# yewzijian/RegTR

Measured on AMD Instinct MI355X. Metric: point-cloud pairs/sec (3DMatch ~20k pts), higher is better.
Workload: dtype f32 (f16-pair split, 22-bit operands)

## Files before the change

### regtr_amd/csrc/block_tail.hip

```cpp
#include "common.h"
#include "mfma_operands.h"

namespace {


constexpr int MO_WAVES = 4;
constexpr int MO_ROWS_WAVE = 512;
constexpr int MO_ROWS_WG = MO_WAVES * MO_ROWS_WAVE;

template <int KC, bool INFOLD, bool ROWDIV>
__global__ void __launch_bounds__(MO_WAVES* RG_WAVE, 4) k_moments(const float* __restrict__ A, int lda, const float2* __restrict__ stats,
                                                               float slope, const float* __restrict__ row_div, int k_valid,
                                                               const int* __restrict__ seg_off, int n_chunks,
                                                               double* __restrict__ partial, float* __restrict__ pivot)
{
    constexpr int K = 32 * KC, NTILE = KC * (KC + 1) / 2;
    __shared__ double red[K * K + K];
    const int cloud = blockIdx.y, chunk = blockIdx.x;
    const int c_end = seg_off[cloud + 1];
    const int wg_begin = seg_off[cloud] + chunk * MO_ROWS_WG;
    if (wg_begin >= c_end) return;
    const int lane = rg_lane(), wave = __builtin_amdgcn_readfirstlane(threadIdx.x >> 6);
    const int half = lane >> 5, ch = lane & 31;
    const bool ch_ok = ch < k_valid;
    const int chc = ch_ok ? ch : 0;
    const int w_begin = wg_begin + wave * MO_ROWS_WAVE, w_end = min(c_end, w_begin + MO_ROWS_WAVE);
    float mu[KC], rs[KC];
#pragma unroll
    for (int c = 0; c < KC; c++) {
        mu[c] = 0.f; rs[c] = 1.f;
        if (INFOLD) { const float2 s = stats[(size_t)cloud * K + 32 * c + chc]; mu[c] = s.x; rs[c] = s.y; }
    }
    float pv[KC];
    {
        const int r0 = seg_off[cloud];
        const long long n_c = c_end - r0;
        float v16[16][KC], d16[ROWDIV ? 16 : 1];
#pragma unroll
        for (int i = 0; i < 16; i++) {
            const int row = r0 + (int)(((2 * i + 1) * n_c) >> 5);
#pragma unroll
            for (int c = 0; c < KC; c++) v16[i][c] = A[(size_t)row * lda + 32 * c + chc];
            if (ROWDIV) d16[i] = row_div[row];
        }
#pragma unroll
        for (int c = 0; c < KC; c++) {
            float acc16 = 0.f, lo = 3.0e38f, hi = -3.0e38f;
#pragma unroll
            for (int i = 0; i < 16; i++) {
                float v = v16[i][c];
                if (ROWDIV) v = v / d16[ROWDIV ? i : 0];
                if (INFOLD) { const float u = (v - mu[c]) * rs[c]; v = fmaxf(u, u * slope); }
                acc16 += v; lo = fminf(lo, v); hi = fmaxf(hi, v);
            }
            pv[c] = ch_ok ? (acc16 - lo - hi) * (1.f / 14.f) : 0.f;
        }
    }
    floatx16 acc[NTILE];
    float s1[KC];
#pragma unroll
    for (int t = 0; t < NTILE; t++)
#pragma unroll
        for (int r = 0; r < 16; r++) acc[t][r] = 0.f;
#pragma unroll
    for (int c = 0; c < KC; c++) s1[c] = 0.f;
    constexpr int SUB = 16;
    constexpr int DS = ROWDIV ? SUB : 1;
    auto load = [&](float (&xv)[SUB][KC], float (&dv)[DS], int base) {
#pragma unroll
        for (int s = 0; s < SUB; s++) {
            const int row = base + 2 * s + half;
            const int rcl = row < w_end ? row : w_end - 1;
            const float* ap = A + (size_t)rcl * lda + chc;
#pragma unroll
            for (int c = 0; c < KC; c++) xv[s][c] = ap[32 * c];
            if (ROWDIV) dv[s] = row_div[rcl];
        }
    };
    auto consume = [&](const float (&xv)[SUB][KC], const float (&dv)[DS], int base) {
#pragma unroll
        for (int s = 0; s < SUB; s++) {
            const bool ok = base + 2 * s + half < w_end && ch_ok;
            float x[KC];
#pragma unroll
            for (int c = 0; c < KC; c++) {
                float v = xv[s][c];
                if (ROWDIV) v = v / dv[ROWDIV ? s : 0];
                if (INFOLD) { const float u = (v - mu[c]) * rs[c]; v = fmaxf(u, u * slope); }
                x[c] = ok ? v - pv[c] : 0.f;
                s1[c] += x[c];
            }
            int t = 0;
#pragma unroll
            for (int ta = 0; ta < KC; ta++)
#pragma unroll
                for (int tb = ta; tb < KC; tb++, t++)
                    acc[t] = __builtin_amdgcn_mfma_f32_32x32x2f32(x[ta], x[tb], acc[t], 0, 0, 0);
        }
    };
    float xa[SUB][KC], xb[SUB][KC], da[DS], db[DS];
    if (w_begin < w_end) load(xa, da, w_begin);
    for (int base = w_begin; base < w_end; base += 4 * SUB) {
        load(xb, db, base + 2 * SUB);
        consume(xa, da, base);
        load(xa, da, base + 4 * SUB);
        consume(xb, db, base + 2 * SUB);
    }
    for (int w = 0; w < MO_WAVES; w++) {
        if (wave == w && w_begin < w_end) {
            int t = 0;
#pragma unroll
            for (int ta = 0; ta < KC; ta++)
#pragma unroll
                for (int tb = ta; tb < KC; tb++, t++)
#pragma unroll
                    for (int r = 0; r < 16; r++) {
                        const int a = 32 * ta + (r & 3) + 8 * (r >> 2) + 4 * half, b = 32 * tb + ch;
                        const double v = (w == 0 ? 0.0 : red[a * K + b]) + (double)acc[t][r];
                        red[a * K + b] = v;
                    }
#pragma unroll
            for (int c = 0; c < KC; c++) {
                const double v = (double)s1[c] + (double)__shfl_xor(s1[c], 32, RG_WAVE);
                if (half == 0) red[K * K + 32 * c + ch] = (w == 0 ? 0.0 : red[K * K + 32 * c + ch]) + v;
            }
        }
        __syncthreads();
    }
    const int kv = k_valid;
    double* out = partial + ((size_t)cloud * n_chunks + chunk) * (kv * kv + kv);
    for (int i = threadIdx.x; i < kv * kv + kv; i += MO_WAVES * RG_WAVE) {
        int src = K * K + (i - kv * kv);
        if (i < kv * kv) { const int a = i / kv, b = i - a * kv; src = a * K + b; }
        out[i] = red[src];
    }
    if (chunk == 0 && wave == 0 && half == 0 && ch_ok) {
#pragma unroll
        for (int c = 0; c < KC; c++) pivot[(size_t)cloud * kv + 32 * c + ch] = pv[c];
    }
}

template <int K>
__device__ void bt_prepare_source(const double* __restrict__ partial, int n_chunks_total, int n_valid, int n_rows, int cloud,
                                  const float* __restrict__ W_kn, int N, int col0, float eps, double* cov ,
                                  double2* quad , uint16_t* __restrict__ planes, float* __restrict__ in_mean,
                                  float2* __restrict__ out_stats, const float* __restrict__ pivot)
{
    const double inv_n = 1.0 / (double)n_rows;
    for (int i = threadIdx.x; i < K * K + K; i += blockDim.x) {
        int src = i;
        if (i < K * K) {
            const int a = i / K, b = i - a * K;
            if ((a >> 5) > (b >> 5)) src = b * K + a;
        }
        double s = 0.0;
        for (int c = 0; c < n_valid; c++) s += partial[((size_t)cloud * n_chunks_total + c) * (K * K + K) + src];
        cov[i] = s * inv_n;
    }
    __syncthreads();
    for (int i = threadIdx.x; i < K * K; i += blockDim.x) {
        const int a = i / K, b = i - a * K;
        cov[i] -= cov[K * K + a] * cov[K * K + b];
    }
    __syncthreads();
    if (threadIdx.x < K) {
        cov[K * K + threadIdx.x] += (double)pivot[(size_t)cloud * K + threadIdx.x];
        if (col0 == 0) in_mean[(size_t)cloud * K + threadIdx.x] = (float)cov[K * K + threadIdx.x];
    }
    __syncthreads();
    const int j = col0 + (threadIdx.x & 63), h = threadIdx.x >> 6;
    float wj[K];
#pragma unroll
    for (int a = 0; a < K; a++) wj[a] = W_kn[(size_t)a * N + j];
    double mean = 0.0, var = 0.0;
#pragma unroll 1
    for (int a = h * (K / 4); a < (h + 1) * (K / 4); a++) {
        double t = 0.0;
#pragma unroll
        for (int b = 0; b < K; b++) t += cov[a * K + b] * (double)wj[b];
        const double wa = (double)W_kn[(size_t)a * N + j];
        mean += cov[K * K + a] * wa;
        var += wa * t;
    }
    quad[threadIdx.x] = make_double2(mean, var);
    __syncthreads();
    {
        const int c = threadIdx.x & 63;
        const double2 q0 = quad[c], q1 = quad[64 + c], q2 = quad[128 + c], q3 = quad[192 + c];
        mean = (q0.x + q1.x) + (q2.x + q3.x);
        var = (q0.y + q1.y) + (q2.y + q3.y);
    }
    if (var < 0.0) var = 0.0;
    const float rstd = (float)(1.0 / sqrt(var + (double)eps));
    if (out_stats && h == 0) out_stats[(size_t)cloud * N + j] = make_float2((float)mean, rstd);
    uint16_t* row = planes + ((size_t)cloud * 3 * N + j) * K;
    for (int k = h * (K / 4); k < (h + 1) * (K / 4); k += 2) {
        unsigned p0, p1, p2;
        rg_split2(W_kn[(size_t)k * N + j] * rstd, W_kn[(size_t)(k + 1) * N + j] * rstd, p0, p1, p2);
        *(unsigned*)(row + k) = p0;
        *(unsigned*)(row + (size_t)N * K + k) = p1;
        *(unsigned*)(row + (size_t)2 * N * K + k) = p2;
    }
    __syncthreads();
}

template <int K1, int K2>
__global__ void __launch_bounds__(256) k_tail_prepare(const double* __restrict__ part1, const double* __restrict__ part2,
                                                      const int* __restrict__ seg_off, int n_chunks, const float* __restrict__ W1,
                                                      const float* __restrict__ W2, int N, float eps, uint16_t* __restrict__ planes1,
                                                      uint16_t* __restrict__ planes2, float* __restrict__ mean1,
                                                      float* __restrict__ mean2, float2* __restrict__ out_stats, int n_clouds,
                                                      const float* __restrict__ pivot1, const float* __restrict__ pivot2)
{
    constexpr int KM = K1 > K2 ? K1 : K2;
    __shared__ double cov[KM * KM + KM];
    __shared__ double2 quad[256];
    const int cloud = blockIdx.x, col0 = blockIdx.y * 64;
    const int n = seg_off[cloud + 1] - seg_off[cloud];
    if (n <= 0) {
        if (out_stats && threadIdx.x < 64) {
            out_stats[(size_t)cloud * N + col0 + threadIdx.x] = make_float2(0.f, 0.f);
            if (K2 > 0) out_stats[((size_t)n_clouds + cloud) * N + col0 + threadIdx.x] = make_float2(0.f, 0.f);
        }
        return;
    }
    const int n_valid = (n + MO_ROWS_WG - 1) / MO_ROWS_WG;
    bt_prepare_source<K1>(part1, n_chunks, n_valid, n, cloud, W1, N, col0, eps, cov, quad, planes1, mean1, out_stats, pivot1);
    if constexpr (K2 > 0)
        bt_prepare_source<K2>(part2, n_chunks, n_valid, n, cloud, W2, N, col0, eps, cov, quad, planes2, mean2,
                              out_stats ? out_stats + (size_t)n_clouds * N : nullptr, pivot2);
}

constexpr int TS_WAVES = 8;
constexpr int TS_ROWS = 32 * TS_WAVES;

struct TailArgs {
    const float* A1; const float* A2; float* Y;
    const float2* a1_stats;
    const float* row_div1;
    const float* mean1; const float* mean2;
    const uint16_t* planes1; const uint16_t* planes2;
    const int* seg_off; const int4* tile_info;
    int M, N, lda1, lda2, ldy, n_seg;
    float a1_slope, slope;
};

template <int KT> __device__ __forceinline__ unsigned ts_swz(unsigned n)
{
    constexpr int CPR = 2 * KT;
    return CPR == 2 ? 0u : (CPR == 4 ? ((n >> 2) & 3u) : (CPR == 8 ? ((n >> 1) & 7u) : (n & 15u)));
}

template <int KT, int NB>
__device__ __forceinline__ void ts_copy_planes(const uint16_t* __restrict__ src , size_t plane,
                                               unsigned char* dst, int t)
{
    constexpr int CPR = 2 * KT, K = 16 * KT, NDMA = 3 * NB * CPR / RG_WAVE;
    static_assert(3 * NB * CPR % RG_WAVE == 0, "whole DMA instructions");
    const int wave = __builtin_amdgcn_readfirstlane(t >> 6), lane = t & 63;
#pragma unroll 1
    for (int q0 = 0; q0 < NDMA; q0 += TS_WAVES) {
        const int q = q0 + wave;
        if (q < NDMA) {
            const int sidx = q * RG_WAVE + lane;
            const int p = sidx / (NB * CPR), rem = sidx - p * (NB * CPR), n = rem / CPR, cs = rem - n * CPR;
            __builtin_amdgcn_global_load_lds((const void*)(src + (size_t)p * plane + (size_t)n * K + (((unsigned)cs ^ ts_swz<KT>((unsigned)n)) * 8)),
                                             (rg_lds_ptr)(dst + (size_t)q * 1024), 16, 0, 0);
        }
    }
}

template <int KT1, int KT2, int NT, int NPASS, bool FOLD1>
__global__ void __launch_bounds__(TS_WAVES* RG_WAVE, NT <= 2 ? 4 : 2) k_tail_strip(TailArgs g)
{
    constexpr int K1 = 16 * KT1, K2 = 16 * KT2, NB = 32 * NT * NPASS, KT2A = KT2 > 0 ? KT2 : 1;
    extern __shared__ __align__(16) unsigned char Ws[];
    unsigned char* Ws2 = Ws + (size_t)3 * NB * K1 * 2;
    const int t = threadIdx.x, lane = t & 63, l31 = lane & 31, hi = lane >> 5;
    const int wave = __builtin_amdgcn_readfirstlane(t >> 6);
    const int N = g.N, n0 = blockIdx.y * NB;
    const int m0 = blockIdx.x * TS_ROWS, r0 = m0 + 32 * wave;
    const int row = r0 + l31;
    const bool row_ok = row < g.M;
    const int rc = row_ok ? row : g.M - 1;

    float4 raw1[KT1][2], raw2[KT2A][2];
    float div1 = 1.f;
    {
        const float* ap = g.A1 + (size_t)rc * g.lda1 + 8 * hi;
#pragma unroll
        for (int ks = 0; ks < KT1; ks++) { raw1[ks][0] = *(const float4*)(ap + 16 * ks); raw1[ks][1] = *(const float4*)(ap + 16 * ks + 4); }
        if constexpr (KT2 > 0) {
            const float* bp = g.A2 + (size_t)rc * g.lda2 + 8 * hi;
#pragma unroll
            for (int ks = 0; ks < KT2; ks++) { raw2[ks][0] = *(const float4*)(bp + 16 * ks); raw2[ks][1] = *(const float4*)(bp + 16 * ks + 4); }
        }
        if (!FOLD1 && g.row_div1) div1 = g.row_div1[rc];
    }
    const int4 ti = g.tile_info[blockIdx.x];
    const int s_lo = ti.x, s_hi = ti.y;
    ts_copy_planes<KT1, NB>(g.planes1 + ((size_t)s_lo * 3 * N + n0) * K1, (size_t)N * K1, Ws, t);
    if constexpr (KT2 > 0) ts_copy_planes<KT2, NB>(g.planes2 + ((size_t)s_lo * 3 * N + n0) * K2, (size_t)N * K2, Ws2, t);
    const int my_seg = s_lo == s_hi ? s_lo : rg_find_segment(g.seg_off, g.n_seg, rc);
    __syncthreads();

    {
        const float* mp = g.mean1 + (size_t)my_seg * K1 + 8 * hi;
        if constexpr (FOLD1) {
            const float2* sp = g.a1_stats + (size_t)my_seg * K1 + 8 * hi;
#pragma unroll
            for (int ks = 0; ks < KT1; ks++)
#pragma unroll
                for (int h = 0; h < 2; h++) {
                    const float4 sa = *(const float4*)(sp + 16 * ks + 4 * h), sb = *(const float4*)(sp + 16 * ks + 4 * h + 2);
                    const float4 m = *(const float4*)(mp + 16 * ks + 4 * h);
                    float4 v = raw1[ks][h];
                    float u;
                    u = (v.x - sa.x) * sa.y; v.x = row_ok ? fmaxf(u, u * g.a1_slope) - m.x : 0.f;
                    u = (v.y - sa.z) * sa.w; v.y = row_ok ? fmaxf(u, u * g.a1_slope) - m.y : 0.f;
                    u = (v.z - sb.x) * sb.y; v.z = row_ok ? fmaxf(u, u * g.a1_slope) - m.z : 0.f;
                    u = (v.w - sb.z) * sb.w; v.w = row_ok ? fmaxf(u, u * g.a1_slope) - m.w : 0.f;
                    raw1[ks][h] = v;
                }
        } else {
#pragma unroll
            for (int ks = 0; ks < KT1; ks++)
#pragma unroll
                for (int h = 0; h < 2; h++) {
                    const float4 m = *(const float4*)(mp + 16 * ks + 4 * h);
                    float4 v = raw1[ks][h];
                    if (g.row_div1) { v.x = v.x / div1; v.y = v.y / div1; v.z = v.z / div1; v.w = v.w / div1; }
                    v.x = row_ok ? v.x - m.x : 0.f; v.y = row_ok ? v.y - m.y : 0.f; v.z = row_ok ? v.z - m.z : 0.f; v.w = row_ok ? v.w - m.w : 0.f;
                    raw1[ks][h] = v;
                }
        }
        if constexpr (KT2 > 0) {
            const float* mq = g.mean2 + (size_t)my_seg * K2 + 8 * hi;
#pragma unroll
            for (int ks = 0; ks < KT2; ks++)
#pragma unroll
                for (int h = 0; h < 2; h++) {
                    const float4 m = *(const float4*)(mq + 16 * ks + 4 * h);
                    float4 v = raw2[ks][h];
                    v.x = row_ok ? v.x - m.x : 0.f; v.y = row_ok ? v.y - m.y : 0.f; v.z = row_ok ? v.z - m.z : 0.f; v.w = row_ok ? v.w - m.w : 0.f;
                    raw2[ks][h] = v;
                }
        }
    }
    auto frag = [&](const float4 (&r)[2], bf16x8 (&fa)[3]) {
        unsigned w[4][3];
        rg_split2(r[0].x, r[0].y, w[0]);
        rg_split2(r[0].z, r[0].w, w[1]);
        rg_split2(r[1].x, r[1].y, w[2]);
        rg_split2(r[1].z, r[1].w, w[3]);
#pragma unroll
        for (int p = 0; p < 3; p++) fa[p] = __builtin_bit_cast(bf16x8, make_uint4(w[0][p], w[1][p], w[2][p], w[3][p]));
    };
    unsigned f1_off[KT1], f2_off[KT2A];
#pragma unroll
    for (int ks = 0; ks < KT1; ks++) f1_off[ks] = (unsigned)l31 * (K1 * 2) + (((unsigned)(2 * ks + hi)) ^ ts_swz<KT1>((unsigned)l31)) * 16u;
    if constexpr (KT2 > 0) {
#pragma unroll
        for (int ks = 0; ks < KT2; ks++) f2_off[ks] = (unsigned)l31 * (K2 * 2) + (((unsigned)(2 * ks + hi)) ^ ts_swz<KT2A>((unsigned)l31)) * 16u;
    }

    const int rbase = r0 + 4 * hi;
    for (int sg = s_lo; sg <= s_hi; sg++) {
        if (sg > s_lo) {
            __syncthreads();
            ts_copy_planes<KT1, NB>(g.planes1 + ((size_t)sg * 3 * N + n0) * K1, (size_t)N * K1, Ws, t);
            if constexpr (KT2 > 0) ts_copy_planes<KT2, NB>(g.planes2 + ((size_t)sg * 3 * N + n0) * K2, (size_t)N * K2, Ws2, t);
            __syncthreads();
        }
        const int c_lo = sg == s_lo ? ti.z : g.seg_off[sg], c_hi = min(sg == s_lo ? ti.w : g.seg_off[sg + 1], g.M);
#pragma unroll 1
        for (int ps = 0; ps < NPASS; ps++) {
            const int cb = 32 * NT * ps;
            floatx16 acc[NT];
#pragma unroll
            for (int j = 0; j < NT; j++)
#pragma unroll
                for (int r = 0; r < 16; r++) acc[j][r] = 0.f;
#define TS_STEP(FA, WS_, OFF, KK)                                                                                            \
            _Pragma("unroll") for (int j = 0; j < NT; j++) {                                                                   \
                bf16x8 fb[3];                                                                                                  \
                _Pragma("unroll") for (int p = 0; p < 3; p++)                                                                  \
                    fb[p] = __builtin_bit_cast(bf16x8, *(const uint4*)(WS_ + (size_t)(p * NB + cb + 32 * j) * (KK * 2) + OFF)); \
                acc[j] = __builtin_amdgcn_mfma_f32_32x32x16_bf16(FA[2], fb[0], acc[j], 0, 0, 0);                               \
                acc[j] = __builtin_amdgcn_mfma_f32_32x32x16_bf16(FA[1], fb[1], acc[j], 0, 0, 0);                               \
                acc[j] = __builtin_amdgcn_mfma_f32_32x32x16_bf16(FA[0], fb[2], acc[j], 0, 0, 0);                               \
                acc[j] = __builtin_amdgcn_mfma_f32_32x32x16_bf16(FA[1], fb[0], acc[j], 0, 0, 0);                               \
                acc[j] = __builtin_amdgcn_mfma_f32_32x32x16_bf16(FA[0], fb[1], acc[j], 0, 0, 0);                               \
                acc[j] = __builtin_amdgcn_mfma_f32_32x32x16_bf16(FA[0], fb[0], acc[j], 0, 0, 0);                               \
            }
#pragma unroll
            for (int ks = 0; ks < KT1; ks++) { bf16x8 fa[3]; frag(raw1[ks], fa); TS_STEP(fa, Ws, f1_off[ks], K1) }
            if constexpr (KT2 > 0) {
#pragma unroll
                for (int ks = 0; ks < KT2; ks++) { bf16x8 fa[3]; frag(raw2[ks], fa); TS_STEP(fa, Ws2, f2_off[ks], K2) }
            }
#undef TS_STEP
            int rb = rbase;
            asm volatile("" : "+v"(rb));
#pragma unroll
            for (int j = 0; j < NT; j++) {
                const int col = n0 + cb + 32 * j + l31;
#pragma unroll
                for (int r = 0; r < 16; r++) {
                    const int rw = rb + (r & 3) + 8 * (r >> 2);
                    const float v = acc[j][r];
                    if (rw >= c_lo && rw < c_hi) g.Y[(size_t)rw * g.ldy + col] = fmaxf(v, v * g.slope);
                }
            }
        }
    }
}

int bt_chunks(int max_len) { return rg_cdiv(max_len > 0 ? max_len : 1, MO_ROWS_WG); }
size_t bt_align(size_t b) { return (b + 255) & ~(size_t)255; }

}

extern "C" {

int regtr_block_tail_supported(int M, int N, int K1, int K2)
{
    return (M >= 0 && ((K1 == 32 && K2 == 64 && N == 128) || (K1 == 16 && K2 == 0 && N == 64))) ? 1 : 0;
}

size_t regtr_block_tail_ws_bytes(int n_clouds, int max_len, int N, int K1, int K2)
{
    if (n_clouds < 1 || !regtr_block_tail_supported(0, N, K1, K2)) return 0;
    const size_t nc = (size_t)bt_chunks(max_len);
    return bt_align(n_clouds * nc * (K1 * K1 + K1) * 8) + bt_align(n_clouds * nc * (K2 * K2 + K2) * 8) +
           bt_align((size_t)n_clouds * 3 * N * K1 * 2) + bt_align((size_t)n_clouds * 3 * N * K2 * 2) +
           2 * (bt_align((size_t)n_clouds * K1 * 4) + bt_align((size_t)n_clouds * K2 * 4));
}

int regtr_block_tail(const float* A1, int lda1, const float* a1_stats, float a1_slope, const float* row_div1, const float* A2, int lda2,
                     const float* W1, const float* W2, const int* seg_off, int n_clouds, int max_len, const void* tile_info,
                     int M, int N, int K1, int K2, float eps, float slope, float* Y, int ldy, void* ws, size_t ws_bytes,
                     float* out_stats, void* stream)
{
    if (!A1 || !W1 || !seg_off || !tile_info || !Y || !ws || n_clouds < 1 || max_len < 0) return RG_ERR_ARG;
    if (!regtr_block_tail_supported(M, N, K1, K2) || lda1 < K1 || ldy < N || (lda1 % 4)) return RG_ERR_ARG;
    if (K2 > 0 && (!A2 || !W2 || !a1_stats || row_div1 || lda2 < K2 || (lda2 % 4) || (uintptr_t)A2 % 16)) return RG_ERR_ARG;
    if (K2 == 0 && (A2 || W2 || a1_stats || !row_div1)) return RG_ERR_ARG;
    if (((uintptr_t)A1 | (uintptr_t)a1_stats | (uintptr_t)tile_info | (uintptr_t)ws) % 16) return RG_ERR_ARG;
    if (ws_bytes < regtr_block_tail_ws_bytes(n_clouds, max_len, N, K1, K2)) return RG_ERR_WORKSPACE;
    if (M == 0 || max_len == 0) return RG_OK;
    const int nc = bt_chunks(max_len);
    unsigned char* p = (unsigned char*)ws;
    double* part1 = (double*)p; p += bt_align((size_t)n_clouds * nc * (K1 * K1 + K1) * 8);
    double* part2 = (double*)p; p += bt_align((size_t)n_clouds * nc * (K2 * K2 + K2) * 8);
    uint16_t* planes1 = (uint16_t*)p; p += bt_align((size_t)n_clouds * 3 * N * K1 * 2);
    uint16_t* planes2 = (uint16_t*)p; p += bt_align((size_t)n_clouds * 3 * N * K2 * 2);
    float* mean1 = (float*)p; p += bt_align((size_t)n_clouds * K1 * 4);
    float* mean2 = (float*)p; p += bt_align((size_t)n_clouds * K2 * 4);
    float* pivot1 = (float*)p; p += bt_align((size_t)n_clouds * K1 * 4);
    float* pivot2 = (float*)p;
    hipStream_t st = (hipStream_t)stream;
    const dim3 mgrid(nc, n_clouds), pgrid(n_clouds, N / 64), sgrid(rg_cdiv(M, TS_ROWS), 1);
    TailArgs g{A1, A2, Y, (const float2*)a1_stats, row_div1, mean1, mean2, planes1, planes2, seg_off, (const int4*)tile_info,
               M, N, lda1, lda2, ldy, n_clouds, a1_slope, slope};
    const size_t lds = (size_t)3 * N * (K1 + K2) * 2;
    if (K2 > 0) {
        k_moments<1, true, false><<<mgrid, MO_WAVES * RG_WAVE, 0, st>>>(A1, lda1, (const float2*)a1_stats, a1_slope, nullptr, K1, seg_off, nc, part1, pivot1);
        k_moments<2, false, false><<<mgrid, MO_WAVES * RG_WAVE, 0, st>>>(A2, lda2, nullptr, 0.f, nullptr, K2, seg_off, nc, part2, pivot2);
        k_tail_prepare<32, 64><<<pgrid, 256, 0, st>>>(part1, part2, seg_off, nc, W1, W2, N, eps, planes1, planes2, mean1, mean2,
                                                      (float2*)out_stats, n_clouds, pivot1, pivot2);
        if (!rg_allow_dynamic_lds<k_tail_strip<2, 4, 2, 2, true>>(lds)) return RG_ERR_ARG;
        k_tail_strip<2, 4, 2, 2, true><<<sgrid, TS_WAVES * RG_WAVE, lds, st>>>(g);
    } else {
        k_moments<1, false, true><<<mgrid, MO_WAVES * RG_WAVE, 0, st>>>(A1, lda1, nullptr, 0.f, row_div1, K1, seg_off, nc, part1, pivot1);
        k_tail_prepare<16, 0><<<pgrid, 256, 0, st>>>(part1, nullptr, seg_off, nc, W1, nullptr, N, eps, planes1, nullptr, mean1, nullptr,
                                                     (float2*)out_stats, n_clouds, pivot1, nullptr);
        if (!rg_allow_dynamic_lds<k_tail_strip<1, 0, 2, 1, false>>(lds)) return RG_ERR_ARG;
        k_tail_strip<1, 0, 2, 1, false><<<sgrid, TS_WAVES * RG_WAVE, lds, st>>>(g);
    }
    RG_RETURN_IF_LAUNCH_FAILED();
    return RG_OK;
}


}
```

Measured before the change: 2290.

## Stage moment inputs through LDS with float4 loads and parallel cross-wave reduction

The moments kernel now loads rows as coalesced float4 vectors into a per-wave LDS stage, applying the normalisation transform once per element, and then reads MFMA operands from LDS. The serial wave-by-wave double reduction is replaced by parking accumulators in LDS and having each wave reduce one slice across waves in parallel. The prepare kernel switches to one 512-thread block per cloud with register-blocked covariance quadratic forms. This trades extra LDS traffic and more LDS use for fewer strided global loads and less serialized reduction, and it hardcodes the column count (k_valid removed).

```diff
diff --git a/regtr_amd/csrc/block_tail.hip b/regtr_amd/csrc/block_tail.hip
--- a/regtr_amd/csrc/block_tail.hip
+++ b/regtr_amd/csrc/block_tail.hip
@@ -8,53 +8,96 @@
 constexpr int MO_ROWS_WAVE = 512;
 constexpr int MO_ROWS_WG = MO_WAVES * MO_ROWS_WAVE;
 
+__device__ __forceinline__ void mo_wave_sync()
+{
+    __builtin_amdgcn_fence(__ATOMIC_RELEASE, "wavefront");
+    __builtin_amdgcn_wave_barrier();
+    __builtin_amdgcn_fence(__ATOMIC_ACQUIRE, "wavefront");
+}
+
 template <int KC, bool INFOLD, bool ROWDIV>
-__global__ void __launch_bounds__(MO_WAVES* RG_WAVE, 4) k_moments(const float* __restrict__ A, int lda, const float2* __restrict__ stats,
-                                                               float slope, const float* __restrict__ row_div, int k_valid,
+__global__ void __launch_bounds__(MO_WAVES* RG_WAVE, KC == 1 ? 4 : 3) k_moments(const float* __restrict__ A, int lda, const float2* __restrict__ stats,
+                                                               float slope, const float* __restrict__ row_div,
                                                                const int* __restrict__ seg_off, int n_chunks,
                                                                double* __restrict__ partial, float* __restrict__ pivot)
 {
+    static_assert(!ROWDIV || KC == 1, "the row_div form has 16 columns");
     constexpr int K = 32 * KC, NTILE = KC * (KC + 1) / 2;
-    __shared__ double red[K * K + K];
+    constexpr int KV = ROWDIV ? 16 : K;
+    constexpr int CPR = KV / 4, RPI = RG_WAVE / CPR;
+    constexpr int NLD = 8, SUBR = NLD * RPI;
+    constexpr int GRP = 8 / KC;
+    constexpr int STAGE_F = SUBR * KV, PARK_F = NTILE * 16 * RG_WAVE, WAVE_F = STAGE_F > PARK_F ? STAGE_F : PARK_F;
+    __shared__ __align__(16) float lds[MO_WAVES * WAVE_F];
+    __shared__ double s1_park[MO_WAVES * K];
     const int cloud = blockIdx.y, chunk = blockIdx.x;
-    const int c_end = seg_off[cloud + 1];
-    const int wg_begin = seg_off[cloud] + chunk * MO_ROWS_WG;
+    const int r0 = seg_off[cloud], c_end = seg_off[cloud + 1];
+    const int wg_begin = r0 + chunk * MO_ROWS_WG;
     if (wg_begin >= c_end) return;
     const int lane = rg_lane(), wave = __builtin_amdgcn_readfirstlane(threadIdx.x >> 6);
     const int half = lane >> 5, ch = lane & 31;
-    const bool ch_ok = ch < k_valid;
-    const int chc = ch_ok ? ch : 0;
+    const bool ch_ok = ch < KV;
+    const int chr = ch & (KV - 1);
+    const int lrow = lane / CPR, lcol = 4 * (lane % CPR);
     const int w_begin = wg_begin + wave * MO_ROWS_WAVE, w_end = min(c_end, w_begin + MO_ROWS_WAVE);
-    float mu[KC], rs[KC];
-#pragma unroll
-    for (int c = 0; c < KC; c++) {
-        mu[c] = 0.f; rs[c] = 1.f;
-        if (INFOLD) { const float2 s = stats[(size_t)cloud * K + 32 * c + chc]; mu[c] = s.x; rs[c] = s.y; }
-    }
+    float* stage = lds + wave * WAVE_F;
+    float mu[4], rs[4];
+#pragma unroll
+    for (int q = 0; q < 4; q++) { mu[q] = 0.f; rs[q] = 1.f; }
+    if (INFOLD) {
+        const float4* sp = (const float4*)(stats + (size_t)cloud * K + lcol);
+        const float4 sa = sp[0], sb = sp[1];
+        mu[0] = sa.x; rs[0] = sa.y; mu[1] = sa.z; rs[1] = sa.w; mu[2] = sb.x; rs[2] = sb.y; mu[3] = sb.z; rs[3] = sb.w;
+    }
+    auto xform = [&](float4 v, float d) {
+        float x[4] = {v.x, v.y, v.z, v.w};
+#pragma unroll
+        for (int q = 0; q < 4; q++) {
+            if (ROWDIV) x[q] = x[q] / d;
+            if (INFOLD) { const float u = (x[q] - mu[q]) * rs[q]; x[q] = fmaxf(u, u * slope); }
+        }
+        return make_float4(x[0], x[1], x[2], x[3]);
+    };
+    float4 buf[NLD];
+    float dv[ROWDIV ? NLD : 1];
+    auto load = [&](int base) {
+#pragma unroll
+        for (int j = 0; j < NLD; j++) {
+            const int row = base + j * RPI + lrow;
+            const int rcl = row < w_end ? row : w_end - 1;
+            buf[j] = *(const float4*)(A + (size_t)rcl * lda + lcol);
+            if (ROWDIV) dv[j] = row_div[rcl];
+        }
+    };
+    if (w_begin < w_end) load(w_begin);
     float pv[KC];
-    {
-        const int r0 = seg_off[cloud];
+#pragma unroll
+    for (int c = 0; c < KC; c++) pv[c] = 0.f;
+    if (w_begin < w_end) {
         const long long n_c = c_end - r0;
-        float v16[16][KC], d16[ROWDIV ? 16 : 1];
-#pragma unroll
-        for (int i = 0; i < 16; i++) {
-            const int row = r0 + (int)(((2 * i + 1) * n_c) >> 5);
-#pragma unroll
-            for (int c = 0; c < KC; c++) v16[i][c] = A[(size_t)row * lda + 32 * c + chc];
-            if (ROWDIV) d16[i] = row_div[row];
-        }
+        constexpr int NS = 16 * CPR / RG_WAVE;
+        float4 sv[NS];
+        float sd[NS];
+#pragma unroll
+        for (int j = 0; j < NS; j++) {
+            const int row = r0 + (int)(((2 * (j * RPI + lrow) + 1) * n_c) >> 5);
+            sv[j] = *(const float4*)(A + (size_t)row * lda + lcol);
+            sd[j] = ROWDIV ? row_div[row] : 1.f;
+        }
+#pragma unroll
+        for (int j = 0; j < NS; j++) *(float4*)(stage + (j * RPI + lrow) * KV + lcol) = xform(sv[j], sd[j]);
+        mo_wave_sync();
 #pragma unroll
         for (int c = 0; c < KC; c++) {
             float acc16 = 0.f, lo = 3.0e38f, hi = -3.0e38f;
 #pragma unroll
             for (int i = 0; i < 16; i++) {
-                float v = v16[i][c];
-                if (ROWDIV) v = v / d16[ROWDIV ? i : 0];
-                if (INFOLD) { const float u = (v - mu[c]) * rs[c]; v = fmaxf(u, u * slope); }
+                const float v = stage[i * KV + 32 * c + chr];
                 acc16 += v; lo = fminf(lo, v); hi = fmaxf(hi, v);
             }
             pv[c] = ch_ok ? (acc16 - lo - hi) * (1.f / 14.f) : 0.f;
         }
+        mo_wave_sync();
     }
     floatx16 acc[NTILE];
     float s1[KC];
@@ -64,170 +107,198 @@
         for (int r = 0; r < 16; r++) acc[t][r] = 0.f;
 #pragma unroll
     for (int c = 0; c < KC; c++) s1[c] = 0.f;
-    constexpr int SUB = 16;
-    constexpr int DS = ROWDIV ? SUB : 1;
-    auto load = [&](float (&xv)[SUB][KC], float (&dv)[DS], int base) {
-#pragma unroll
-        for (int s = 0; s < SUB; s++) {
-            const int row = base + 2 * s + half;
-            const int rcl = row < w_end ? row : w_end - 1;
-            const float* ap = A + (size_t)rcl * lda + chc;
-#pragma unroll
-            for (int c = 0; c < KC; c++) xv[s][c] = ap[32 * c];
-            if (ROWDIV) dv[s] = row_div[rcl];
-        }
-    };
-    auto consume = [&](const float (&xv)[SUB][KC], const float (&dv)[DS], int base) {
-#pragma unroll
-        for (int s = 0; s < SUB; s++) {
-            const bool ok = base + 2 * s + half < w_end && ch_ok;
-            float x[KC];
-#pragma unroll
-            for (int c = 0; c < KC; c++) {
-                float v = xv[s][c];
-                if (ROWDIV) v = v / dv[ROWDIV ? s : 0];
-                if (INFOLD) { const float u = (v - mu[c]) * rs[c]; v = fmaxf(u, u * slope); }
-                x[c] = ok ? v - pv[c] : 0.f;
-                s1[c] += x[c];
-            }
-            int t = 0;
-#pragma unroll
-            for (int ta = 0; ta < KC; ta++)
-#pragma unroll
-                for (int tb = ta; tb < KC; tb++, t++)
-                    acc[t] = __builtin_amdgcn_mfma_f32_32x32x2f32(x[ta], x[tb], acc[t], 0, 0, 0);
-        }
-    };
-    float xa[SUB][KC], xb[SUB][KC], da[DS], db[DS];
-    if (w_begin < w_end) load(xa, da, w_begin);
-    for (int base = w_begin; base < w_end; base += 4 * SUB) {
-        load(xb, db, base + 2 * SUB);
-        consume(xa, da, base);
-        load(xa, da, base + 4 * SUB);
-        consume(xb, db, base + 2 * SUB);
-    }
-    for (int w = 0; w < MO_WAVES; w++) {
-        if (wave == w && w_begin < w_end) {
-            int t = 0;
-#pragma unroll
-            for (int ta = 0; ta < KC; ta++)
-#pragma unroll
-                for (int tb = ta; tb < KC; tb++, t++)
-#pragma unroll
-                    for (int r = 0; r < 16; r++) {
-                        const int a = 32 * ta + (r & 3) + 8 * (r >> 2) + 4 * half, b = 32 * tb + ch;
-                        const double v = (w == 0 ? 0.0 : red[a * K + b]) + (double)acc[t][r];
-                        red[a * K + b] = v;
+    for (int base = w_begin; base < w_end; base += SUBR) {
+#pragma unroll
+        for (int j = 0; j < NLD; j++) *(float4*)(stage + (j * RPI + lrow) * KV + lcol) = xform(buf[j], ROWDIV ? dv[ROWDIV ? j : 0] : 1.f);
+        mo_wave_sync();
+        if (base + SUBR < w_end) load(base + SUBR);
+        for (int s0 = 0; s0 < SUBR / 2 && base + 2 * s0 < w_end; s0 += GRP) {
+            float xv[GRP][KC];
+#pragma unroll
+            for (int s = 0; s < GRP; s++)
+#pragma unroll
+                for (int c = 0; c < KC; c++) xv[s][c] = stage[(2 * (s0 + s) + half) * KV + 32 * c + chr];
+#pragma unroll
+            for (int s = 0; s < GRP; s++)
+#pragma unroll
+                for (int c = 0; c < KC; c++) asm volatile("" : "+v"(xv[s][c]));
+#pragma unroll
+            for (int s = s0; s < s0 + GRP; s++) {
+                const bool ok = base + 2 * s + half < w_end && ch_ok;
+                float x[KC];
+#pragma unroll
+                for (int c = 0; c < KC; c++) {
+                    x[c] = ok ? xv[s - s0][c] - pv[c] : 0.f;
+                    s1[c] += x[c];
+                }
+                int t = 0;
+#pragma unroll
+                for (int ta = 0; ta < KC; ta++)
+#pragma unroll
+                    for (int tb = ta; tb < KC; tb++, t++)
+                        acc[t] = __builtin_amdgcn_mfma_f32_32x32x2f32(x[ta], x[tb], acc[t], 0, 0, 0);
+            }
+        }
+        mo_wave_sync();
+    }
+    if (w_begin < w_end) {
+#pragma unroll
+        for (int t = 0; t < NTILE; t++)
+#pragma unroll
+            for (int g = 0; g < 4; g++)
+                ((float4*)stage)[(t * 4 + g) * RG_WAVE + lane] = make_float4(acc[t][4 * g], acc[t][4 * g + 1], acc[t][4 * g + 2], acc[t][4 * g + 3]);
+#pragma unroll
+        for (int c = 0; c < KC; c++) {
+            const double v = (double)s1[c] + (double)__shfl_xor(s1[c], 32, RG_WAVE);
+            if (half == 0) s1_park[wave * K + 32 * c + ch] = v;
+        }
+    }
+    __syncthreads();
+    const int n_act = min(MO_WAVES, (c_end - wg_begin + MO_ROWS_WAVE - 1) / MO_ROWS_WAVE);
+    double* out = partial + ((size_t)cloud * n_chunks + chunk) * (KV * KV + KV);
+    {
+        const int g = wave;
+        int t = 0;
+#pragma unroll
+        for (int ta = 0; ta < KC; ta++)
+#pragma unroll
+            for (int tb = ta; tb < KC; tb++, t++) {
+                double sum[4] = {0.0, 0.0, 0.0, 0.0};
+#pragma unroll
+                for (int w = 0; w < MO_WAVES; w++)
+                    if (w < n_act) {
+                        const float4 v = ((const float4*)(lds + w * WAVE_F))[(t * 4 + g) * RG_WAVE + lane];
+                        sum[0] += (double)v.x; sum[1] += (double)v.y; sum[2] += (double)v.z; sum[3] += (double)v.w;
                     }
-#pragma unroll
-            for (int c = 0; c < KC; c++) {
-                const double v = (double)s1[c] + (double)__shfl_xor(s1[c], 32, RG_WAVE);
-                if (half == 0) red[K * K + 32 * c + ch] = (w == 0 ? 0.0 : red[K * K + 32 * c + ch]) + v;
-            }
-        }
-        __syncthreads();
-    }
-    const int kv = k_valid;
-    double* out = partial + ((size_t)cloud * n_chunks + chunk) * (kv * kv + kv);
-    for (int i = threadIdx.x; i < kv * kv + kv; i += MO_WAVES * RG_WAVE) {
-        int src = K * K + (i - kv * kv);
-        if (i < kv * kv) { const int a = i / kv, b = i - a * kv; src = a * K + b; }
-        out[i] = red[src];
+                const int a = 32 * ta + 8 * g + 4 * half, b = 32 * tb + ch;
+#pragma unroll
+                for (int q = 0; q < 4; q++)
+                    if (a + q < KV && b < KV) out[(size_t)(a + q) * KV + b] = sum[q];
+            }
+    }
+    if (threadIdx.x < KV) {
+        double s = 0.0;
+        for (int w = 0; w < n_act; w++) s += s1_park[w * K + threadIdx.x];
+        out[KV * KV + threadIdx.x] = s;
     }
     if (chunk == 0 && wave == 0 && half == 0 && ch_ok) {
 #pragma unroll
-        for (int c = 0; c < KC; c++) pivot[(size_t)cloud * kv + 32 * c + ch] = pv[c];
-    }
-}
+        for (int c = 0; c < KC; c++) pivot[(size_t)cloud * KV + 32 * c + ch] = pv[c];
+    }
+}
+
+constexpr int PR_THREADS = 512;
+constexpr int PR_MAX_N = 128;
 
 template <int K>
 __device__ void bt_prepare_source(const double* __restrict__ partial, int n_chunks_total, int n_valid, int n_rows, int cloud,
-                                  const float* __restrict__ W_kn, int N, int col0, float eps, double* cov ,
+                                  const float* __restrict__ W_kn, int N, float eps, double* cov ,
                                   double2* quad , uint16_t* __restrict__ planes, float* __restrict__ in_mean,
                                   float2* __restrict__ out_stats, const float* __restrict__ pivot)
 {
+    constexpr int NEL = K * K + K, NE = (NEL + PR_THREADS - 1) / PR_THREADS;
     const double inv_n = 1.0 / (double)n_rows;
-    for (int i = threadIdx.x; i < K * K + K; i += blockDim.x) {
-        int src = i;
-        if (i < K * K) {
-            const int a = i / K, b = i - a * K;
-            if ((a >> 5) > (b >> 5)) src = b * K + a;
-        }
-        double s = 0.0;
-        for (int c = 0; c < n_valid; c++) s += partial[((size_t)cloud * n_chunks_total + c) * (K * K + K) + src];
-        cov[i] = s * inv_n;
-    }
-    __syncthreads();
-    for (int i = threadIdx.x; i < K * K; i += blockDim.x) {
+    {
+        const double* pc = partial + (size_t)cloud * n_chunks_total * NEL;
+        int src[NE];
+        double s[NE];
+#pragma unroll
+        for (int e = 0; e < NE; e++) {
+            const int i = threadIdx.x + e * PR_THREADS;
+            src[e] = i < NEL ? i : 0;
+            if (i < K * K) {
+                const int a = i / K, b = i - a * K;
+                if ((a >> 5) > (b >> 5)) src[e] = b * K + a;
+            }
+            s[e] = 0.0;
+        }
+        for (int c = 0; c < n_valid; c++)
+#pragma unroll
+            for (int e = 0; e < NE; e++) s[e] += pc[(size_t)c * NEL + src[e]];
+#pragma unroll
+        for (int e = 0; e < NE; e++) {
+            const int i = threadIdx.x + e * PR_THREADS;
+            if (i < NEL) cov[i] = s[e] * inv_n;
+        }
+    }
+    __syncthreads();
+    for (int i = threadIdx.x; i < K * K; i += PR_THREADS) {
         const int a = i / K, b = i - a * K;
         cov[i] -= cov[K * K + a] * cov[K * K + b];
     }
     __syncthreads();
     if (threadIdx.x < K) {
         cov[K * K + threadIdx.x] += (double)pivot[(size_t)cloud * K + threadIdx.x];
-        if (col0 == 0) in_mean[(size_t)cloud * K + threadIdx.x] = (float)cov[K * K + threadIdx.x];
-    }
-    __syncthreads();
-    const int j = col0 + (threadIdx.x & 63), h = threadIdx.x >> 6;
-    float wj[K];
-#pragma unroll
-    for (int a = 0; a < K; a++) wj[a] = W_kn[(size_t)a * N + j];
-    double mean = 0.0, var = 0.0;
+        in_mean[(size_t)cloud * K + threadIdx.x] = (float)cov[K * K + threadIdx.x];
+    }
+    __syncthreads();
+    for (int item = threadIdx.x; item < 4 * N; item += PR_THREADS) {
+        const int h = item / N, j = item - h * N;
+        float wj[K];
+#pragma unroll
+        for (int a = 0; a < K; a++) wj[a] = W_kn[(size_t)a * N + j];
+        double mean = 0.0, var = 0.0;
 #pragma unroll 1
-    for (int a = h * (K / 4); a < (h + 1) * (K / 4); a++) {
-        double t = 0.0;
-#pragma unroll
-        for (int b = 0; b < K; b++) t += cov[a * K + b] * (double)wj[b];
-        const double wa = (double)W_kn[(size_t)a * N + j];
-        mean += cov[K * K + a] * wa;
-        var += wa * t;
-    }
-    quad[threadIdx.x] = make_double2(mean, var);
-    __syncthreads();
-    {
-        const int c = threadIdx.x & 63;
-        const double2 q0 = quad[c], q1 = quad[64 + c], q2 = quad[128 + c], q3 = quad[192 + c];
-        mean = (q0.x + q1.x) + (q2.x + q3.x);
-        var = (q0.y + q1.y) + (q2.y + q3.y);
-    }
-    if (var < 0.0) var = 0.0;
-    const float rstd = (float)(1.0 / sqrt(var + (double)eps));
-    if (out_stats && h == 0) out_stats[(size_t)cloud * N + j] = make_float2((float)mean, rstd);
-    uint16_t* row = planes + ((size_t)cloud * 3 * N + j) * K;
-    for (int k = h * (K / 4); k < (h + 1) * (K / 4); k += 2) {
-        unsigned p0, p1, p2;
-        rg_split2(W_kn[(size_t)k * N + j] * rstd, W_kn[(size_t)(k + 1) * N + j] * rstd, p0, p1, p2);
-        *(unsigned*)(row + k) = p0;
-        *(unsigned*)(row + (size_t)N * K + k) = p1;
-        *(unsigned*)(row + (size_t)2 * N * K + k) = p2;
+        for (int a0 = h * (K / 4); a0 < (h + 1) * (K / 4); a0 += 4) {
+            double t[4] = {0.0, 0.0, 0.0, 0.0};
+#pragma unroll
+            for (int b = 0; b < K; b++)
+#pragma unroll
+                for (int u = 0; u < 4; u++) t[u] = fma(cov[(a0 + u) * K + b], (double)wj[b], t[u]);
+#pragma unroll
+            for (int u = 0; u < 4; u++) {
+                const double wa = (double)W_kn[(size_t)(a0 + u) * N + j];
+                mean = fma(cov[K * K + a0 + u], wa, mean);
+                var = fma(wa, t[u], var);
+            }
+        }
+        quad[item] = make_double2(mean, var);
+    }
+    __syncthreads();
+    for (int item = threadIdx.x; item < 4 * N; item += PR_THREADS) {
+        const int h = item / N, j = item - h * N;
+        const double2 q0 = quad[j], q1 = quad[N + j], q2 = quad[2 * N + j], q3 = quad[3 * N + j];
+        const double mean = (q0.x + q1.x) + (q2.x + q3.x);
+        double var = (q0.y + q1.y) + (q2.y + q3.y);
+        if (var < 0.0) var = 0.0;
+        const float rstd = (float)(1.0 / sqrt(var + (double)eps));
+        if (out_stats && h == 0) out_stats[(size_t)cloud * N + j] = make_float2((float)mean, rstd);
+        uint16_t* row = planes + ((size_t)cloud * 3 * N + j) * K;
+        for (int k = h * (K / 4); k < (h + 1) * (K / 4); k += 2) {
+            unsigned p0, p1, p2;
+            rg_split2(W_kn[(size_t)k * N + j] * rstd, W_kn[(size_t)(k + 1) * N + j] * rstd, p0, p1, p2);
+            *(unsigned*)(row + k) = p0;
+            *(unsigned*)(row + (size_t)N * K + k) = p1;
+            *(unsigned*)(row + (size_t)2 * N * K + k) = p2;
+        }
     }
     __syncthreads();
 }
 
 template <int K1, int K2>
-__global__ void __launch_bounds__(256) k_tail_prepare(const double* __restrict__ part1, const double* __restrict__ part2,
-                                                      const int* __restrict__ seg_off, int n_chunks, const float* __restrict__ W1,
-                                                      const float* __restrict__ W2, int N, float eps, uint16_t* __restrict__ planes1,
-                                                      uint16_t* __restrict__ planes2, float* __restrict__ mean1,
-                                                      float* __restrict__ mean2, float2* __restrict__ out_stats, int n_clouds,
-                                                      const float* __restrict__ pivot1, const float* __restrict__ pivot2)
+__global__ void __launch_bounds__(PR_THREADS) k_tail_prepare(const double* __restrict__ part1, const double* __restrict__ part2,
+                                                             const int* __restrict__ seg_off, int n_chunks, const float* __restrict__ W1,
+                                                             const float* __restrict__ W2, int N, float eps, uint16_t* __restrict__ planes1,
+                                                             uint16_t* __restrict__ planes2, float* __restrict__ mean1,
+                                                             float* __restrict__ mean2, float2* __restrict__ out_stats, int n_clouds,
+                                                             const float* __restrict__ pivot1, const float* __restrict__ pivot2)
 {
     constexpr int KM = K1 > K2 ? K1 : K2;
     __shared__ double cov[KM * KM + KM];
-    __shared__ double2 quad[256];
-    const int cloud = blockIdx.x, col0 = blockIdx.y * 64;
+    __shared__ double2 quad[4 * PR_MAX_N];
+    const int cloud = blockIdx.x;
     const int n = seg_off[cloud + 1] - seg_off[cloud];
     if (n <= 0) {
-        if (out_stats && threadIdx.x < 64) {
-            out_stats[(size_t)cloud * N + col0 + threadIdx.x] = make_float2(0.f, 0.f);
-            if (K2 > 0) out_stats[((size_t)n_clouds + cloud) * N + col0 + threadIdx.x] = make_float2(0.f, 0.f);
+        if (out_stats && threadIdx.x < N) {
+            out_stats[(size_t)cloud * N + threadIdx.x] = make_float2(0.f, 0.f);
+            if (K2 > 0) out_stats[((size_t)n_clouds + cloud) * N + threadIdx.x] = make_float2(0.f, 0.f);
         }
         return;
     }
     const int n_valid = (n + MO_ROWS_WG - 1) / MO_ROWS_WG;
-    bt_prepare_source<K1>(part1, n_chunks, n_valid, n, cloud, W1, N, col0, eps, cov, quad, planes1, mean1, out_stats, pivot1);
+    bt_prepare_source<K1>(part1, n_chunks, n_valid, n, cloud, W1, N, eps, cov, quad, planes1, mean1, out_stats, pivot1);
     if constexpr (K2 > 0)
-        bt_prepare_source<K2>(part2, n_chunks, n_valid, n, cloud, W2, N, col0, eps, cov, quad, planes2, mean2,
+        bt_prepare_source<K2>(part2, n_chunks, n_valid, n, cloud, W2, N, eps, cov, quad, planes2, mean2,
                               out_stats ? out_stats + (size_t)n_clouds * N : nullptr, pivot2);
 }
 
@@ -460,20 +531,20 @@
     float* pivot1 = (float*)p; p += bt_align((size_t)n_clouds * K1 * 4);
     float* pivot2 = (float*)p;
     hipStream_t st = (hipStream_t)stream;
-    const dim3 mgrid(nc, n_clouds), pgrid(n_clouds, N / 64), sgrid(rg_cdiv(M, TS_ROWS), 1);
+    const dim3 mgrid(nc, n_clouds), pgrid(n_clouds), sgrid(rg_cdiv(M, TS_ROWS), 1);
     TailArgs g{A1, A2, Y, (const float2*)a1_stats, row_div1, mean1, mean2, planes1, planes2, seg_off, (const int4*)tile_info,
                M, N, lda1, lda2, ldy, n_clouds, a1_slope, slope};
     const size_t lds = (size_t)3 * N * (K1 + K2) * 2;
     if (K2 > 0) {
-        k_moments<1, true, false><<<mgrid, MO_WAVES * RG_WAVE, 0, st>>>(A1, lda1, (const float2*)a1_stats, a1_slope, nullptr, K1, seg_off, nc, part1, pivot1);
-        k_moments<2, false, false><<<mgrid, MO_WAVES * RG_WAVE, 0, st>>>(A2, lda2, nullptr, 0.f, nullptr, K2, seg_off, nc, part2, pivot2);
-        k_tail_prepare<32, 64><<<pgrid, 256, 0, st>>>(part1, part2, seg_off, nc, W1, W2, N, eps, planes1, planes2, mean1, mean2,
+        k_moments<1, true, false><<<mgrid, MO_WAVES * RG_WAVE, 0, st>>>(A1, lda1, (const float2*)a1_stats, a1_slope, nullptr, seg_off, nc, part1, pivot1);
+        k_moments<2, false, false><<<mgrid, MO_WAVES * RG_WAVE, 0, st>>>(A2, lda2, nullptr, 0.f, nullptr, seg_off, nc, part2, pivot2);
+        k_tail_prepare<32, 64><<<pgrid, PR_THREADS, 0, st>>>(part1, part2, seg_off, nc, W1, W2, N, eps, planes1, planes2, mean1, mean2,
                                                       (float2*)out_stats, n_clouds, pivot1, pivot2);
         if (!rg_allow_dynamic_lds<k_tail_strip<2, 4, 2, 2, true>>(lds)) return RG_ERR_ARG;
         k_tail_strip<2, 4, 2, 2, true><<<sgrid, TS_WAVES * RG_WAVE, lds, st>>>(g);
     } else {
-        k_moments<1, false, true><<<mgrid, MO_WAVES * RG_WAVE, 0, st>>>(A1, lda1, nullptr, 0.f, row_div1, K1, seg_off, nc, part1, pivot1);
-        k_tail_prepare<16, 0><<<pgrid, 256, 0, st>>>(part1, nullptr, seg_off, nc, W1, nullptr, N, eps, planes1, nullptr, mean1, nullptr,
+        k_moments<1, false, true><<<mgrid, MO_WAVES * RG_WAVE, 0, st>>>(A1, lda1, nullptr, 0.f, row_div1, seg_off, nc, part1, pivot1);
+        k_tail_prepare<16, 0><<<pgrid, PR_THREADS, 0, st>>>(part1, nullptr, seg_off, nc, W1, nullptr, N, eps, planes1, nullptr, mean1, nullptr,
                                                      (float2*)out_stats, n_clouds, pivot1, nullptr);
         if (!rg_allow_dynamic_lds<k_tail_strip<1, 0, 2, 1, false>>(lds)) return RG_ERR_ARG;
         k_tail_strip<1, 0, 2, 1, false><<<sgrid, TS_WAVES * RG_WAVE, lds, st>>>(g);
```

Measured after the change: 2284 (median of 2 runs). No clear change (-0.3%).
